# w111liang222/lidar-slam-detection

Measured on AMD Instinct MI355X. Metric: registered points/sec (120k-pt scan vs 1e7-pt map, full iterate-to-converge), higher is better.
Workload: dtype f32 per-point geometry / f64 transforms and reductions

## Files before the change

include/lio_hip.h:

```cpp
#ifndef LIO_HIP_H_
#define LIO_HIP_H_

#include <stdint.h>

#ifdef __cplusplus
extern "C" {
#endif

#define LIO_OK 0
#define LIO_E_INVALID (-1)
#define LIO_E_CAPACITY (-2)
#define LIO_E_DEVICE (-3)
#define LIO_E_STATE (-4)

typedef struct lio_map lio_map;
typedef struct lio_scan lio_scan;
typedef struct lio_engine lio_engine;

const char* lio_last_error(void);
const char* lio_last_warning(void);
int lio_device_count(void);
#define LIO_ABI_VERSION 16
int lio_abi_version(void);
void* lio_pinned_alloc(uint64_t bytes);
void lio_pinned_free(void* p);
uint64_t lio_map_bytes(const lio_map*);

lio_map* lio_map_create(int device, float resolution, uint64_t max_points, uint64_t max_voxels, int stencil);
void lio_map_destroy(lio_map*);
int lio_map_set_stencil(lio_map*, int stencil);
int lio_map_insert(lio_map*, const float* world_xyzi, uint64_t n, double travel);
int lio_map_insert_device(lio_map*, const void* d_world_xyzi, uint64_t n, double travel);
int lio_map_clear(lio_map*);
int lio_map_set_lru(lio_map*, uint64_t capacity_voxels, double max_distance);
int lio_map_lru_stats(lio_map*, uint64_t* n_evicted, uint64_t* n_interleaved);
int lio_map_lru_exact_stats(lio_map*, uint64_t* n_recreated, uint64_t* n_batches_not_followed);
int lio_map_set_tie_mode(lio_map*, int mode);
// ... 175 lines not shown
lio_batch* lio_batch_create_sequences(int device, float resolution, int stencil, uint64_t max_points, uint64_t max_voxels, int n_slots, int n_groups,
                                      uint32_t max_raw, uint32_t max_ds);
int lio_batch_sequences_step(lio_batch*, lio_scan_job* jobs, int n_jobs, double* cov_out);
int lio_batch_fastlio_main(lio_batch*, int* rc_out);
void lio_batch_destroy(lio_batch*);
int lio_batch_process(lio_batch*, lio_scan_job* jobs, int n_jobs);
typedef struct lio_batch_times {
    double downsample_us, knn_us, linearize_us, step_us;
    uint32_t downsample_launches, knn_launches, linearize_launches, step_launches;
    double insert_us;
    uint32_t insert_launches, pad;
} lio_batch_times;
int lio_batch_enable_kernel_timing(lio_batch*, int on);
int lio_batch_kernel_times(lio_batch*, lio_batch_times* out, int reset);
lio_engine* lio_batch_engine(lio_batch*, int group, int slot);
int lio_engine_set_static_map(lio_engine*, int on);

typedef struct lio_ndt lio_ndt;
lio_ndt* lio_ndt_create(int device, float resolution, int search_method, uint64_t max_points, uint64_t max_voxels, uint32_t max_source_points);
void lio_ndt_destroy(lio_ndt*);
int lio_ndt_set_target(lio_ndt*, const float* xyzi, uint64_t n);
int lio_ndt_set_target_device(lio_ndt*, const void* d_xyzi, uint64_t n);
int lio_ndt_num_voxels(lio_ndt*);
int lio_ndt_voxel_at(lio_ndt*, const float p[3], float mean[3], float cinv[9]);
int lio_ndt_linearize(lio_ndt*, lio_scan* source, const double T[16], int update_corr, int with_derivatives, double H[36], double b[6],
                      double* err, uint32_t* n_corr);
int lio_ndt_fitness_score(lio_ndt*, lio_scan* source, const double T[16], double max_range, double* score, uint32_t* n_inliers);
int lio_ndt_overlap_score(lio_ndt*, lio_scan* source, const double relpose[16], double max_range, double xy_range, double min_z, double* score,
                          double* inlier_ratio);
typedef struct lio_ndt_times {
// ... 388 lines not shown
```

lidar-slam-detection_amd/csrc/batch.hip:

```cpp
#include <sched.h>
#include <stdlib.h>

#include <chrono>
#include <deque>
#include <vector>

#include "eskf.h"
#include "lio_common.h"

using namespace lio;

int engine_resume_update(lio_engine* e, const double* x_now26, const double* x_prop26, const double* P_prop, int i, int converge, int t);
void engine_count_passes(lio_engine* e, int* n_pass, int* n_knn);
int engine_joint_register_device(lio_engine* e, const void* d_raw, uint32_t n_raw, double lidar_beg_time, double state26[26], double cov[529]);
struct lio_comm;
extern "C" int lio_comm_world(const lio_comm*);
extern "C" {
int engine_seq_prepare(lio_engine* e, uint32_t n_raw, double lidar_beg_time, int* ekf_inited);
void engine_seq_params(lio_engine* e, double* laser_cov, int* maximum_iter, int* degenerate_detect_en, float* leaf_surf, float* leaf_map, int* static_map,
                       double* travel, double last_pos_lid[3]);
int engine_seq_finish(lio_engine* e, const double x26[26], const double P529[529], int n_ds, int n_pass, int n_knn, int n_eff, int degenerate, int inserted,
                      uint32_t n_add, uint32_t map_err, uint32_t bound);
int engine_seq_resume(lio_engine* e, const double* x_now26, const double* x_prop26, const double* P_prop, int i, int converge, int t);
int engine_seq_has_lru(lio_engine* e);
// ... 15 lines not shown
    MapRef* d_rowmaps = nullptr;
    std::vector<MapRef> rowmap_rows;
    char* d_block = nullptr;
    char* h_block = nullptr;
    size_t block_bytes = 0;
    SlotDesc* d_desc = nullptr;
    SlotDesc* h_desc = nullptr;
    EskfDev* d_ctrl = nullptr;
    EskfDev* h_ctrl = nullptr;
    hipGraphExec_t exec[5] = {nullptr, nullptr, nullptr, nullptr, nullptr};
    const void* graph_table = nullptr;
    int graph_stencil = 0;
    lio_batch_result* h_res = nullptr;
    lio_batch_result* h_res_dev = nullptr;
    std::vector<int> job_of_slot;
    float4* d_rawbuf = nullptr;
    MapRef* d_maps = nullptr;
    MapRef* h_maps = nullptr;
    SeqDev* d_seq = nullptr;
    SeqDev* h_seq = nullptr;
    std::vector<int> seq_path;
    int any_lru = 0;
    int n_active = 0;
    int launched_passes = 4;
    uint32_t seq = 0;
    uint32_t max_n_raw = 0;
    BatchTimer* bt = nullptr;
};

}

struct lio_batch {
    lio_map* map = nullptr;
    int device = 0;
    int n_slots = 0;
    uint32_t max_raw = 0, max_ds = 0;
    int pred_passes = 4;
    bool broken = false;
    int use_graph = 1;
    int count_touched = 0;
    std::vector<lio_map*> maps;
    lio_comm* comm = nullptr;
    int world = 1;
    int rank = 0;
    int split_ds = 1;
    uint32_t ds_cap = 0;
    uint32_t ds_seen_max = 0;
    bool ds_cap_full = false;
    uint64_t n_ds_cut = 0;
    int (*gather_hook)(void*, const double*, double*, uint32_t, void*) = nullptr;
    void* gather_ctx = nullptr;
    bool joint = false;
    bool sequences = false;
    std::vector<lio_scan_job> fl_jobs;
// ... 55 lines not shown
    ek_begin(c);
}

void group_free(Group& g) {
    for (lio_engine* e : g.eng) lio_engine_destroy(e);
    for (lio_engine* e : g.sub_eng) lio_engine_destroy(e);
    if (g.d_local32) hipFree(g.d_local32);
    if (g.d_gathered) hipFree(g.d_gathered);
    if (g.d_ds_send) hipFree(g.d_ds_send);
    if (g.d_ds_all) hipFree(g.d_ds_all);
    if (g.d_rowmaps) hipFree(g.d_rowmaps);
    for (int k = 0; k < 5; k++)
        if (g.exec[k]) hipGraphExecDestroy(g.exec[k]);
    if (g.d_block) hipFree(g.d_block);
    if (g.d_rawbuf) hipFree(g.d_rawbuf);
    if (g.h_block) hipHostFree(g.h_block);
    if (g.d_seq) hipFree(g.d_seq);
    if (g.h_seq) hipHostFree(g.h_seq);
    if (g.h_res) hipHostFree(g.h_res);
    if (g.stream) hipStreamDestroy(g.stream);
    if (g.bt) {
        if (g.bt->created)
            for (int c = 0; c < BatchTimer::kClasses; c++)
                for (int i = 0; i < BatchTimer::kPool; i++) { hipEventDestroy(g.bt->ev[c][i][0]); hipEventDestroy(g.bt->ev[c][i][1]); }
        delete g.bt;
    }
}

const float4* stage_host_raw(lio_batch* b, Group& g, int slot, const lio_scan_job& job, int* rc) {
    *rc = LIO_OK;
// ... 84 lines not shown
            if (b->ds_cap == 0) {
                const char* k = getenv("LIO_JOINT_DS_CAP");
                const uint32_t want = k ? (uint32_t)strtoul(k, nullptr, 10) : ((ds_bound / 4u + 1023u) & ~1023u);
                b->ds_cap = std::min(ds_bound, std::max(k ? 1u : 4096u, want));
            }
            const uint32_t cap = b->ds_cap_full ? ds_bound : b->ds_cap;
            rc = p2plane_batch_exchange_ds(b->comm, b->world, b->gather_hook, b->gather_ctx, g.stream, g.d_desc, B, per, s0, s1, cap, g.d_ds_send, g.d_ds_all);
            if (rc == LIO_OK && s0 > 0) rc = scan_begin_rows(g.stream, g.d_desc, s0);
            if (rc == LIO_OK && s1 < B) rc = scan_begin_rows(g.stream, g.d_desc + s1, B - s1);
            if (rc != LIO_OK) return rc;
        } else {
            if (bt) bt->begin(0);
            rc = vg_downsample_batch(g.stream, g.d_desc, B, b->max_raw, b->max_ds, 0.5f, passes);
            if (bt) bt->end(0);
            if (rc != LIO_OK) return rc;
        }
        if (b->joint) {
            rc = p2plane_batch_share(g.stream, g.d_desc, B, M, ds_bound);
            if (rc == LIO_OK) rc = scan_begin_rows(g.stream, g.d_desc + B, B * (M - 1));
            if (rc != LIO_OK) return rc;
            return p2plane_batch_update_joint(b->maps.data(), M, b->comm, b->world, b->gather_hook, b->gather_ctx, g.stream, g.d_desc, B, ds_bound, 5, g.d_local32, g.d_gathered, bt,
                                              rowmaps);
        }
        return p2plane_batch_update(b->map, g.stream, g.d_desc, B, ds_bound, 5, bt, bt ? b->count_touched : 0);
    };
    if (!b->use_graph || timed || b->joint) return enqueue(timed ? g.bt : nullptr);
    if (g.graph_table != b->map->table || g.graph_stencil != b->map->stencil.n) {
        for (int k = 0; k < 5; k++)
            if (g.exec[k]) { hipGraphExecDestroy(g.exec[k]); g.exec[k] = nullptr; }
        g.graph_table = b->map->table;
// ... 44 lines not shown
    if (hipSetDevice(map->device) != hipSuccess) { set_error("lio_batch_create: no HIP device %d", map->device); return nullptr; }
    lio_batch* b = new lio_batch();
    b->map = map;
    b->device = map->device;
    b->n_slots = n_slots;
    b->max_raw = max_raw;
    b->max_ds = max_ds;
    b->maps.assign(maps, maps + n_maps);
    b->comm = comm;
    b->world = comm ? lio_comm_world(comm) : 1;
    b->rank = comm ? lio_comm_rank(comm) : 0;
    { const char* k = getenv("LIO_JOINT_SPLIT_DS"); b->split_ds = (k && k[0] == '0') ? 0 : 1; }
    b->joint = n_maps > 1 || comm != nullptr;
    b->groups.resize(n_groups);
    { const char* k = getenv("LIO_BATCH_GRAPH"); b->use_graph = (k && k[0] == '0') ? 0 : 1; }
    bool ok = true;
    const int M = n_maps;
    for (Group& g : b->groups) ok = ok && hipStreamCreateWithFlags(&g.stream, hipStreamNonBlocking) == hipSuccess;
    for (Group& g : b->groups) {
        g.job_of_slot.assign(n_slots, -1);
        const size_t desc_bytes = sizeof(SlotDesc) * (size_t)n_slots * (size_t)M;
        g.block_bytes = desc_bytes + sizeof(EskfDev) * (size_t)n_slots;
        ok = ok && hipMalloc(reinterpret_cast<void**>(&g.d_block), g.block_bytes) == hipSuccess;
        ok = ok && hipHostMalloc(reinterpret_cast<void**>(&g.h_block), g.block_bytes, hipHostMallocDefault) == hipSuccess;
        if (ok) {
            g.d_desc = reinterpret_cast<SlotDesc*>(g.d_block);
            g.h_desc = reinterpret_cast<SlotDesc*>(g.h_block);
            g.d_ctrl = reinterpret_cast<EskfDev*>(g.d_block + desc_bytes);
            g.h_ctrl = reinterpret_cast<EskfDev*>(g.h_block + desc_bytes);
        }
        ok = ok && hipHostMalloc(reinterpret_cast<void**>(&g.h_res), sizeof(lio_batch_result) * n_slots, hipHostMallocMapped) == hipSuccess;
        ok = ok && hipHostGetDevicePointer(reinterpret_cast<void**>(&g.h_res_dev), g.h_res, 0) == hipSuccess;
        if (b->joint) {
            ok = ok && hipMalloc(reinterpret_cast<void**>(&g.d_local32), sizeof(double) * 32 * n_slots) == hipSuccess;
            ok = ok && hipMalloc(reinterpret_cast<void**>(&g.d_gathered), sizeof(double) * 32 * n_slots * (size_t)b->world) == hipSuccess;
        }
        if (!ok) break;
        memset(g.h_block, 0, g.block_bytes);
        memset(g.h_res, 0, sizeof(lio_batch_result) * n_slots);
        ok = hipMemset(g.d_block, 0, g.block_bytes) == hipSuccess;
        for (int s = 0; s < n_slots && ok; s++) {
            lio_engine* e = lio_engine_create_shared(map, max_raw, max_ds);
            if (!e) { ok = false; break; }
            lio_engine_set_flags(e, 1, 0, 0.0, -10.0);
            g.eng.push_back(e);
            fill_desc(g.h_desc[s], lio_engine_scan(e), &g.d_ctrl[s], &g.h_res_dev[s]);
        }
        for (int m = 1; m < M && ok; m++)
            for (int s = 0; s < n_slots && ok; s++) {
                lio_engine* e = lio_engine_create_shared(maps[m], max_raw, max_ds);
                if (!e) { ok = false; break; }
                lio_engine_set_flags(e, 1, 0, 0.0, -10.0);
                g.sub_eng.push_back(e);
                fill_desc(g.h_desc[(size_t)m * n_slots + s], lio_engine_scan(e), &g.d_ctrl[s], nullptr);
            }
        for (int s = 0; s < n_slots && ok && b->joint; s++) {
            std::vector<lio_engine*> others;
            for (int m = 1; m < M; m++) others.push_back(g.sub_eng[(size_t)(m - 1) * n_slots + s]);
            ok = lio_engine_set_joint(g.eng[s], others.empty() ? nullptr : others.data(), (int)others.size(), comm) == LIO_OK;
        }
    }
// ... 84 lines not shown
int lio_batch_kernel_times(lio_batch* b, lio_batch_times* out, int reset) {
    if (!b || !out) return LIO_E_INVALID;
    memset(out, 0, sizeof(*out));
    for (Group& g : b->groups) {
        if (!g.bt) continue;
        out->downsample_us += g.bt->us[0]; out->knn_us += g.bt->us[1]; out->linearize_us += g.bt->us[2]; out->step_us += g.bt->us[3];
        out->downsample_launches += g.bt->launches[0]; out->knn_launches += g.bt->launches[1]; out->linearize_launches += g.bt->launches[2];
        out->step_launches += g.bt->launches[3];
        out->insert_us += g.bt->us[4];
        out->insert_launches += g.bt->launches[4];
        if (reset)
            for (int c = 0; c < BatchTimer::kClasses; c++) { g.bt->us[c] = 0; g.bt->launches[c] = 0; }
    }
    return LIO_OK;
}

lio_engine* lio_batch_engine(lio_batch* b, int group, int slot) {
    if (!b || group < 0 || group >= (int)b->groups.size() || slot < 0 || slot >= b->n_slots) return nullptr;
    return b->groups[group].eng[slot];
}

int lio_batch_process(lio_batch* b, lio_scan_job* jobs, int n_jobs) {
    if (!b || (!jobs && n_jobs) || n_jobs < 0) return LIO_E_INVALID;
    if (b->sequences) { set_error("lio_batch_process: a sequence batch is driven by lio_batch_sequences_step"); return LIO_E_STATE; }
    hipSetDevice(b->device);
    const int B = b->n_slots;
    int next = 0, first_err = 0;
    std::deque<int> inflight;
    std::vector<int> retry;
    auto note = [&](int rc) { if (rc < 0 && !first_err) first_err = rc; };
// ... 562 lines not shown
```

lidar-slam-detection_amd/csrc/knn.hip:

```cpp
#include "hashgrid.h"
#include "knn_dev.h"
#include "lio_common.h"
#include "refsel.h"

namespace lio {

#ifndef LIO_KNN_G
#define LIO_KNN_G 16
#endif
#ifndef LIO_KNN_U
#define LIO_KNN_U 4
#endif
#ifndef LIO_KNN_WAVES
#define LIO_KNN_WAVES 6
#endif
#ifndef LIO_KNN_PRUNE
#define LIO_KNN_PRUNE 1
#endif
#ifndef LIO_KNN_STAT
#define LIO_KNN_STAT 1
#endif
#ifndef LIO_KNN_WAVES_BATCH
#define LIO_KNN_WAVES_BATCH 7
#endif
// ... 255 lines not shown
__device__ __noinline__ bool cand_tie_less(const Cand& a, const Cand& b, const float4* __restrict__ pool) {
    if (a.id == b.id) return false;
    if (a.id == kNoIdx || b.id == kNoIdx) return a.id < b.id;
    const float4 pa = pool[a.id], pb = pool[b.id];
    if (pa.x != pb.x) return pa.x < pb.x;
    if (pa.y != pb.y) return pa.y < pb.y;
    if (pa.z != pb.z) return pa.z < pb.z;
    return a.id < b.id;
}
__device__ inline bool cand_less(const Cand& a, const Cand& b, const float4* __restrict__ pool) {
    if (a.d2 != b.d2) return a.d2 < b.d2;
    return cand_tie_less(a, b, pool);
}


template <int KM, int MODE, bool COUNT = false, class PoseFill>
__device__ __forceinline__ void knn_body(const Slot* __restrict__ table, uint32_t mask, const float4* __restrict__ pool,
                                         float inv_res, const StencilArgs& st, PoseFill fill, const float4* __restrict__ queries,
                                         uint32_t n_host, const ScanDev* __restrict__ sd, float4* __restrict__ world_out,
                                         float4* __restrict__ nn_pts, uint32_t nn_stride, int32_t* __restrict__ nn_cnt,
                                         MapDev* md, uint32_t* __restrict__ n_tie, uint32_t* __restrict__ tie_list) {
    __shared__ GroupLds lds[kGPB];
    const int tid = threadIdx.x;
    const int grp = tid / kG, gl = tid % kG;
    const int lane = tid & 63;
    GroupLds& g = lds[grp];
    const uint32_t n = sd ? sd->n_ds : n_host;
    const unsigned long long gmask = ((1ull << kG) - 1ull) << (lane - gl);
    __shared__ uint32_t stat_s[256 / 64];
    if (tid < 256 / 64) stat_s[tid] = 0;
    uint32_t touched = 0;
    uint32_t fresh = 0;
    uint32_t* const bits = COUNT ? md->touch_bits : nullptr;
    const float res = 1.0f / inv_res;
    const uint32_t b1_bits = __float_as_uint(0.0625f * res * res), b2_bits = __float_as_uint(0.25f * res * res);
    (void)b1_bits; (void)b2_bits;

    const uint32_t nblk = (n + kGPB - 1) / kGPB;
    const uint32_t per_xcd = (nblk + 7u) >> 3;
    const uint32_t wg_per_xcd = gridDim.x >> 3;
    constexpr uint32_t kAhead = 64 / kGPB;
    __shared__ float4 pw_s[64];
    __shared__ PoseArgs pose_s;
    if constexpr (MODE == 0) fill(pose_s);
    uint32_t ahead = kAhead;
    for (uint32_t j = blockIdx.x >> 3; j < per_xcd; j += wg_per_xcd) {
        const uint32_t q0 = ((blockIdx.x & 7u) * per_xcd + j) * kGPB;
        const uint32_t q = q0 + grp;
        const bool active = q < n;
        float4 pw = make_float4(0.f, 0.f, 0.f, 0.f);
        if constexpr (MODE == 0) {
            if (ahead == kAhead) {
                __syncthreads();
                if (tid < 64) {
                    const uint32_t j2 = j + (uint32_t)(tid / kGPB) * wg_per_xcd;
                    const uint32_t q2 = ((blockIdx.x & 7u) * per_xcd + j2) * kGPB + (uint32_t)(tid % kGPB);
                    if (j2 < per_xcd && q2 < n) {
                        float4 w2;
                        body_to_world(pose_s, queries[q2], w2);
                        world_out[q2] = w2;
                        uint32_t t2 = (uint32_t)tid;
                        asm volatile("" : "+v"(t2));
                        pw_s[t2] = w2;
                    }
                }
                __syncthreads();
                ahead = 0;
            }
            if (active) pw = pw_s[ahead * kGPB + grp];
            ahead++;
        } else {
            if (active) pw = queries[q];
        }
        int kx = 0, ky = 0, kz = 0;
        pos2grid(pw.x, pw.y, pw.z, inv_res, kx, ky, kz);
        uint32_t nhit = 0;
        constexpr bool kPrune = LIO_KNN_PRUNE && KM * kG <= 32;
        uint32_t n0 = 0, n01 = 0, total;
// ... 101 lines not shown
        for (int r = 0; r < 6; r++) {
            const uint32_t bd = group_min32(d0);
            const uint32_t bi = group_min32(d0 == bd ? i0d : 0xFFFFFFFFu);
            const bool some = bi != 0xFFFFFFFFu;
            if (r > 0 && some && bd == prev_d) tie = true;
            prev_d = some ? bd : 0xFFFFFFFFu;
            if (gl == r) win = bi;
            if (some && d0 == bd && i0d == bi) {
                d0 = d1; d1 = dd2; dd2 = d3; d3 = d4; d4 = 0xFFFFFFFFu;
                i0d = i1d; i1d = i2d; i2d = i3d; i3d = i4d; i4d = 0xFFFFFFFFu;
                pops++;
            }
        }
        if (group_ballot(pops >= 5 && drop_tie, lane)) tie = true;
        if (active && inrange > 0) {
            if (gl < 5) {
                uint32_t g2 = (uint32_t)gl;
                asm volatile("" : "+v"(g2));
                nn_pts[g2 * nn_stride + q] = (win != 0xFFFFFFFFu) ? pool[win] : make_float4(0.f, 0.f, 0.f, 0.f);
            }
            if (gl == 0) {
                nn_cnt[q] = inrange < 5 ? (int32_t)inrange : 5;
                if (tie) tie_list[atomicAdd(n_tie, 1u)] = q;
            }
        }
        group_lds_sync();
    }
    __shared__ unsigned long long vred[256 / 64];
    if constexpr (LIO_KNN_STAT || COUNT) {
        __syncthreads();
        uint32_t te = threadIdx.x;
        asm volatile("" : "+v"(te));
        if (te < 256 / 64) vred[te] = stat_s[te];
        __syncthreads();
        if (tid == 0) {
            const unsigned long long v = (vred[0] + vred[1]) + (vred[2] + vred[3]);
            if (v) atomicAdd(&md->knn_cand[(blockIdx.x & 63) * 16], v);
        }
// ... 27 lines not shown
                                                  float inv_res, StencilArgs st, PoseArgs pose, const float4* __restrict__ queries,
                                                  uint32_t n_host, const ScanDev* __restrict__ sd, float4* __restrict__ world_out,
                                                  float4* __restrict__ nn_pts, uint32_t nn_stride, int32_t* __restrict__ nn_cnt,
                                                  MapDev* md, uint32_t* __restrict__ n_tie, uint32_t* __restrict__ tie_list) {
    knn_body<KM, MODE>(table, mask, pool, inv_res, st, [&](PoseArgs& P) { if (threadIdx.x == 0) P = pose; }, queries, n_host, sd, world_out, nn_pts, nn_stride, nn_cnt, md,
                       n_tie, tie_list);
}
template <int KM, bool COUNT>
__global__ void LIO_KNN_OCC __launch_bounds__(256, COUNT ? LIO_KNN_WAVES : LIO_KNN_WAVES_BATCH) knn_batch_kernel(const Slot* __restrict__ table, uint32_t mask, const float4* __restrict__ pool,
                                                                       float inv_res, StencilArgs st, const SlotDesc* __restrict__ slots, MapDev* md) {
    const SlotDesc& d = slots[blockIdx.y];
    if (!d.active) return;
    const SlotGateLite sg = slot_gate_lite(d);
    if ((sg.status != EK_RUNNING) | (sg.converge == 0) | (sg.n_ds < d.min_ds)) return;
    const double* __restrict__ x = d.ctrl->x;
    knn_body<KM, 0, COUNT>(table, mask, pool, inv_res, st, [x](PoseArgs& P) { pose_fill_from_state(P, x); }, d.ds_body, sg.n_ds, nullptr, d.ds_world, d.nn_pts,
                                  d.max_ds, d.nn_cnt, md, &d.sd->n_tie, d.tie_list);
}

constexpr int kSelCap = 2560;
struct SelLds {
    uint32_t a_d[kSelCap], a_id[kSelCap], a_seq[kSelCap];
    refsel::Rec list[kSelCap];
    refsel::Rec fin[5 * kMaxStencil + 8];
    uint32_t v_ptr[kMaxStencil], v_cnt[kMaxStencil];
    uint32_t v_first[kMaxStencil + 1];
    uint32_t seg_m[kMaxStencil], seg_base[kMaxStencil + 1], seg_keep[kMaxStencil];
    uint32_t wsum[4];
    uint32_t out_d[8], out_id[8];
    int size;
};

// ... 263 lines not shown
    const SlotGate sg = slot_gate(d);
    if ((sg.status != EK_RUNNING) | (sg.converge == 0) | (sg.n_ds < d.min_ds)) return;
    knn_refsel_body<0>(r.table, r.mask, r.pool, r.pool_seq, r.inv_res, st, sg.pose, d.ds_body, d.nn_pts, d.max_ds, &d.sd->n_tie, d.tie_list, r.md, r.tie_mode, sg.n_ds);
}
template <int KM>
__global__ void __launch_bounds__(256) knn_exact_batch_kernel(const Slot* __restrict__ table, uint32_t mask, const float4* __restrict__ pool,
                                                              float inv_res, StencilArgs st, const SlotDesc* __restrict__ slots, int tie_mode) {
    const SlotDesc& d = slots[blockIdx.y];
    if (!d.active || d.sd->n_tie == 0) return;
    const SlotGate sg = slot_gate(d);
    if ((sg.status != EK_RUNNING) | (sg.converge == 0) | (sg.n_ds < d.min_ds)) return;
    const PoseArgs& pose = sg.pose;
    knn_exact_body<KM, 0>(table, mask, pool, inv_res, st, pose, d.ds_body, d.nn_pts, d.max_ds, &d.sd->n_tie, d.tie_list, tie_mode);
}

int knn_batch_launch(lio_map* m, hipStream_t st, const SlotDesc* d_slots, int n_slots, uint32_t grid_x, int count_touched) {
    static const uint32_t forced = [] { const char* e = getenv("LIO_KNN_GRID"); const int v = e ? atoi(e) : 0; return v >= 8 ? (uint32_t)v : 0u; }();
    uint32_t cap = forced ? forced : (12288u / (uint32_t)(n_slots > 0 ? n_slots : 1));
    if (cap > 2048u) cap = 2048u;
    if (cap < 128u) cap = 128u;
    if (grid_x > cap) grid_x = cap;
    if (grid_x == 0) grid_x = 8;
    const dim3 grid((grid_x + 7u) & ~7u, (uint32_t)n_slots);
    const dim3 gridx(n_slots > 8 ? 8 : 64, (uint32_t)n_slots);
    const int tmode = m->pool_seq ? m->tie_mode : 0;
    const int km = (m->stencil.n + kG - 1) / kG;
    if (count_touched && m->touch_bits) LIO_HIP_TRY(hipMemsetAsync(m->touch_bits, 0, (size_t)((m->pool_cap + 31) / 32) * 4, st));
#define KNNB_LAUNCH(KM)                                                                                                                              \
    do {                                                                                                                                             \
        if (count_touched) hipLaunchKernelGGL((knn_batch_kernel<KM, true>), grid, 256, 0, st, m->table, m->table_mask, m->pool, m->inv_res, m->stencil, d_slots, m->dev); \
// ... 152 lines not shown
```

lidar-slam-detection_amd/csrc/lio_common.h:

```cpp
#pragma once
#include <hip/hip_runtime.h>
#include <stdint.h>
#include <stdio.h>
#include <string.h>

#include "../../include/lio_hip.h"
#include "eskf_dev.h"

struct LruEntry;

namespace lio {

#if defined(__HIP_DEVICE_COMPILE__)
#define LIO_PIN4(r) asm volatile("" : "+v"((r).x), "+v"((r).y), "+v"((r).z), "+v"((r).w))
#define LIO_PIN1(r) asm volatile("" : "+v"(r))
#else
#define LIO_PIN4(r) ((void)(r))
#define LIO_PIN1(r) ((void)(r))
#endif
__host__ __device__ __forceinline__ void pin_loaded(float4& r) { LIO_PIN4(r); }
__host__ __device__ __forceinline__ void pin_loaded(uint4& r) { LIO_PIN4(r); }
__host__ __device__ __forceinline__ void pin_loaded(uint32_t& r) { LIO_PIN1(r); }
__host__ __device__ __forceinline__ void pin_loaded(float& r) { LIO_PIN1(r); }

// ... 91 lines not shown
    uint32_t nblocks;
    uint32_t active;
    uint32_t seq;
    uint32_t max_ds, partial_blocks;
    uint32_t min_ds;
    uint32_t reset_cache;
    ScanDev* sd;
    uint32_t *keys_a, *keys_b, *vals_a, *vals_b, *hist, *blockcnt, *hpos, *longlist, *tie_list;
    float4 *sorted, *ds_body, *ds_world, *nn_pts, *normvec;
    int32_t* nn_cnt;
    uint8_t* selected;
    double* partial;
    uint32_t* host_nds;
    EskfDev* ctrl;
    lio_batch_result* result;
};

struct MapRef {
    Slot* table;
    uint32_t* cap;
    uint32_t* pending;
    float* created;
    float4* pool;
    uint32_t* pool_seq;
    MapDev* md;
    uint32_t* slot_of_point;
    float4* stage;
    unsigned long long pool_cap;
    unsigned long long stamp_base;
    unsigned long long* touch;
// ... 152 lines not shown
constexpr int kMaxPoseList = 64;
struct PoseListArgs {
    int n_poses;
    unsigned long long limit[kMaxPoseList];
    DeltaArgs d[kMaxPoseList];
};
int undistort_poses_launch(hipStream_t stream, const float4* d_in, const uint32_t* d_stamp_us, uint32_t n, float4* d_out, const PoseListArgs& args,
                           uint32_t* d_tile_max);
int undistort_delta_launch(hipStream_t stream, const float4* d_in, const uint32_t* d_stamp_us, uint32_t n, float4* d_out, const DeltaArgs& args);
int undistort_launch(hipStream_t stream, const float4* d_in, const uint32_t* d_stamp_us, uint32_t n, float4* d_out, const ImuPoseDev* d_poses,
                     const UndistortArgs& args, unsigned long long* d_block_min );

int vg_downsample(lio_scan* s, float leaf, int passes );
int vg_downsample_batch(hipStream_t st, const SlotDesc* d_slots, int n_slots, uint32_t max_raw, uint32_t max_ds, float leaf, int passes);
int knn_batch_launch(lio_map* m, hipStream_t st, const SlotDesc* d_slots, int n_slots, uint32_t grid_x, int count_touched);
struct BatchTimer {
    static constexpr int kClasses = 5;
    static constexpr int kPool = 256;
    hipEvent_t ev[kClasses][kPool][2];
    int used[kClasses] = {0, 0, 0, 0, 0};
    double us[kClasses] = {0, 0, 0, 0, 0};
    uint32_t launches[kClasses] = {0, 0, 0, 0, 0};
    bool on = false, created = false;
    hipStream_t stream = nullptr;
    void begin(int c) { if (on && used[c] < kPool) hipEventRecord(ev[c][used[c]][0], stream); }
    void end(int c) { if (on && used[c] < kPool) { hipEventRecord(ev[c][used[c]][1], stream); used[c]++; } }
    void resolve() {
        for (int c = 0; c < kClasses; c++) {
            for (int i = 0; i < used[c]; i++) {
                float ms = 0.f;
// ... 51 lines not shown
```

lidar-slam-detection_amd/python/lsd_amd/capi.py:

```python
import ctypes as C
import os

import numpy as np

_HERE = os.path.dirname(os.path.abspath(__file__))
os.environ.setdefault("GPU_MAX_HW_QUEUES", "8")
LIB_PATH = os.environ.get("LIO_HIP_LIB") or os.path.join(_HERE, "liblio_hip.so")

LIO_OK, LIO_E_INVALID, LIO_E_CAPACITY, LIO_E_DEVICE, LIO_E_STATE = 0, -1, -2, -3, -4
MAIN_FIRST_SCAN, MAIN_SEEDED, MAIN_SKIPPED, MAIN_UPDATED, MAIN_IMU_INIT, MAIN_IDLE = 0, 1, 2, 3, 4, 5

SYMBOLS = [
    "lio_last_warning",
    "lio_last_error", "lio_device_count", "lio_map_bytes",
    "lio_map_create", "lio_map_destroy", "lio_map_set_lru", "lio_map_lru_stats", "lio_map_lru_exact_stats", "lio_map_set_tie_mode", "lio_map_tie_stats", "lio_map_clear", "lio_map_pool_stats", "lio_map_set_stencil", "lio_map_insert", "lio_map_insert_device", "lio_map_stats",
    "lio_abi_version", "lio_pinned_alloc", "lio_pinned_free",
    "lio_map_dump", "lio_map_knn", "lio_map_knn_candidates", "lio_map_knn_touched", "lio_map_knn_unique",
    "lio_scan_create", "lio_scan_destroy", "lio_scan_reset", "lio_scan_upload", "lio_scan_set_device", "lio_scan_undistort_delta", "lio_scan_undistort_poses", "lio_scan_undistort_imu", "lio_scan_download_raw", "lio_scan_voxel_downsample", "lio_scan_voxel_downsample_batch", "lio_scan_set_ds",
    "lio_scan_num_ds", "lio_scan_download_ds", "lio_scan_download_world", "lio_scan_download_match",
    "lio_p2plane_linearize", "lio_scan_set_degeneracy_mode", "lio_p2plane_degeneracy", "lio_engine_set_reduce_hook", "lio_p2plane_rows", "lio_map_incremental", "lio_map_seed",
    "lio_engine_create", "lio_engine_create_shared", "lio_engine_destroy", "lio_engine_map", "lio_engine_scan", "lio_engine_set_state", "lio_engine_get_state",
    "lio_engine_set_cov", "lio_engine_get_cov", "lio_engine_set_flags", "lio_engine_travel", "lio_engine_is_degenerate",
    "lio_engine_update", "lio_engine_pass_log", "lio_engine_process_scan", "lio_engine_process_scan_device", "lio_engine_timings", "lio_engine_flush",
    "lio_engine_enable_timing", "lio_comm_unique_id", "lio_comm_init", "lio_comm_destroy", "lio_comm_rank", "lio_comm_world", "lio_allgather_normal_eq", "lio_comm_stats", "lio_engine_set_joint", "lio_engine_joint_register", "lio_engine_joint_register_device", "lio_allgather_records", "lio_engines_process_batch", "lio_batch_create", "lio_batch_create_joint", "lio_batch_create_sequences", "lio_batch_sequences_step", "lio_batch_fastlio_main", "lio_batch_set_gather_hook", "lio_batch_exchange_stats", "lio_batch_destroy", "lio_batch_process", "lio_batch_engine", "lio_batch_enable_kernel_timing", "lio_batch_kernel_times", "lio_engine_set_static_map", "lio_scan_enable_kernel_timing", "lio_scan_kernel_times",
    "lio_state_boxplus", "lio_state_boxminus",
    "lio_localmap_create", "lio_localmap_destroy", "lio_localmap_add_keyframe", "lio_localmap_num_keyframes", "lio_localmap_update",
    "lio_localmap_download",
    "lio_cloud_create", "lio_cloud_destroy", "lio_cloud_clear", "lio_cloud_size", "lio_cloud_append_scan", "lio_cloud_append_host",
    "lio_cloud_voxel_downsample", "lio_cloud_download", "lio_cloud_scratch_bytes", "lio_cloud_last_times",
    "lio_knn_index_create", "lio_knn_index_destroy", "lio_knn_index_build", "lio_knn_index_query", "lio_knn_index_colour", "lio_knn_index_last_times",
    "lio_ground_default_params", "lio_ground_draw", "lio_ground_create", "lio_ground_destroy", "lio_ground_detect_scan", "lio_ground_detect_host",
    "lio_ground_download_indices", "lio_ground_download_normals", "lio_ground_download_inliers", "lio_ground_download_draws", "lio_ground_last_run",
    "lio_ground_last_times",
    "lio_bev_create", "lio_bev_destroy", "lio_bev_preprocess_host", "lio_bev_preprocess_cloud", "lio_bev_upload_pixels", "lio_bev_convert", "lio_bev_get_info",
    "lio_bev_download_pixel_coords", "lio_bev_download_kept", "lio_bev_download_pixels", "lio_bev_download_nodes", "lio_bev_download_equalised",
    "lio_bev_download_image", "lio_bev_grey_table", "lio_bev_last_times",
    "lio_keyframe_decide", "lio_keyframer_default_params", "lio_keyframer_create", "lio_keyframer_destroy", "lio_keyframer_reset", "lio_keyframer_push_host",
    "lio_keyframer_pending", "lio_keyframer_pop", "lio_radius_outlier_host", "lio_keyframe_filter_host", "lio_keyframer_fitness_host",
    "lio_keyframer_append_local_map_host", "lio_keyframer_download_local_map", "lio_keyframer_last_times",
# ... 262 lines not shown
    sig("lio_comm_stats", cint, vp, C.POINTER(u64), f64p)
    sig("lio_engine_set_joint", cint, vp, C.POINTER(vp), cint, vp)
    sig("lio_engine_joint_register", cint, vp, f32p, u32, dbl, f64p, f64p)
    sig("lio_engine_joint_register_device", cint, vp, vp, u32, dbl, f64p, f64p)
    sig("lio_allgather_records", cint, vp, vp, vp, u32, vp)
    sig("lio_batch_create_joint", vp, C.POINTER(vp), cint, vp, cint, cint, u32, u32)
    sig("lio_batch_set_gather_hook", cint, vp, GATHER_FN, vp, cint, cint)
    sig("lio_batch_exchange_stats", cint, vp, C.POINTER(C.c_uint32), C.POINTER(C.c_uint64), C.POINTER(C.c_uint64))
    sig("lio_batch_create", vp, vp, cint, cint, u32, u32)
    sig("lio_batch_create_sequences", vp, cint, C.c_float, cint, u64, u64, cint, cint, u32, u32)
    sig("lio_batch_sequences_step", cint, vp, C.POINTER(ScanJob), cint, C.POINTER(C.c_double))
    sig("lio_batch_fastlio_main", cint, vp, C.POINTER(cint))
    sig("lio_batch_destroy", None, vp)
    sig("lio_batch_process", cint, vp, C.POINTER(ScanJob), cint)
    sig("lio_batch_engine", vp, vp, cint, cint)
    sig("lio_batch_enable_kernel_timing", cint, vp, cint)
    sig("lio_batch_kernel_times", cint, vp, C.POINTER(BatchTimes), cint)
    sig("lio_engine_set_static_map", cint, vp, cint)
    sig("lio_localmap_create", vp, cint, u64, u32, u32)
    sig("lio_localmap_destroy", None, vp)
    sig("lio_localmap_add_keyframe", cint, vp, f32p, u32, f32p)
    sig("lio_localmap_num_keyframes", cint, vp)
    sig("lio_localmap_update", cint, vp, vp, f64p, dbl, dbl, dbl, flt, C.POINTER(cint), C.POINTER(u32))
    sig("lio_localmap_download", cint, vp, f32p, u32)
    sig("lio_cloud_create", vp, cint, u64)
    sig("lio_cloud_destroy", None, vp)
    sig("lio_cloud_clear", cint, vp)
    sig("lio_cloud_size", cint, vp, C.POINTER(u64))
    sig("lio_cloud_append_scan", cint, vp, vp, f64p, flt, cint, dbl, dbl)
    sig("lio_cloud_append_host", cint, vp, f32p, u64, f64p, flt, cint, dbl, dbl)
# ... 198 lines not shown
```

lidar-slam-detection_amd/python/lsd_amd/lio.py:

```python
import ctypes as C

import numpy as np

from . import capi
from .capi import check, f32, f64, lib, ptr

STATE_DIM = 26
DOF = 23
G_LEN = 9.809


def default_state():
    s = np.zeros(STATE_DIM)
    s[6] = 1.0
    s[10] = 1.0
    s[23] = G_LEN
    return s


def init_cov():
    P = np.eye(23)
    for i in (6, 7, 8, 9, 10, 11):
        P[i, i] = 0.00001
    for i in (15, 16, 17):
# ... 1559 lines not shown
        check(lib().lio_batch_set_gather_hook(self.h, self._gather, None, int(rank), int(world)), "set_gather_hook")

    def exchange_stats(self):
        cap, again, nbytes = C.c_uint32(0), C.c_uint64(0), C.c_uint64(0)
        check(lib().lio_batch_exchange_stats(self.h, C.byref(cap), C.byref(again), C.byref(nbytes)))
        return {"chunk_points": cap.value, "jobs_rerun": again.value, "bytes_per_rank_and_round": nbytes.value}

    def enable_kernel_timing(self, on=True):
        check(lib().lio_batch_enable_kernel_timing(self.h, int(on)))

    def kernel_times(self, reset=True):
        t = capi.BatchTimes()
        check(lib().lio_batch_kernel_times(self.h, C.byref(t), int(reset)))
        return {k: getattr(t, k) for k, _ in t._fields_}

    def engine(self, group, slot):
        h = lib().lio_batch_engine(self.h, group, slot)
        if not h:
            raise capi.LioError("no such slot")
        e = Engine.__new__(Engine)
        e.h = h
        e._own = False
        e.map = self.map
        e.scan = Scan(max_ds=100000, _borrow=lib().lio_engine_scan(h))
        return e

    def process(self, jobs):
        return process_batch(None, jobs, batch=self)


# ... 379 lines not shown
```

Baseline: 5.948 billion.

## Sort KNN queries by Morton order of downsampled points for map locality

Adds a per-slot kernel that computes a 30-bit Morton key for each downsampled scan point and radix-sorts indices in LDS, producing a query permutation. The batch KNN kernel then stages queries in this spatial order and writes results back to the original indices, so neighbouring threads probe nearby hash-grid cells and map points. The aim is better cache reuse and less divergence in map lookups, at the cost of an extra sort launch per scan and an indirection in query loads. Scans larger than the LDS cap fall back to identity order.

```diff
diff --git a/include/lio_hip.h b/include/lio_hip.h
--- a/include/lio_hip.h
+++ b/include/lio_hip.h
@@ -20,7 +20,7 @@
 const char* lio_last_error(void);
 const char* lio_last_warning(void);
 int lio_device_count(void);
-#define LIO_ABI_VERSION 16
+#define LIO_ABI_VERSION 17
 int lio_abi_version(void);
 void* lio_pinned_alloc(uint64_t bytes);
 void lio_pinned_free(void* p);
@@ -226,6 +226,9 @@
 int lio_batch_enable_kernel_timing(lio_batch*, int on);
 int lio_batch_kernel_times(lio_batch*, lio_batch_times* out, int reset);
 lio_engine* lio_batch_engine(lio_batch*, int group, int slot);
+int lio_batch_set_query_order(lio_batch*, int on);
+int lio_batch_query_order(lio_batch*, int group, int slot, uint32_t* out, uint32_t cap);
+uint32_t lio_batch_query_order_cap(void);
 int lio_engine_set_static_map(lio_engine*, int on);
 
 typedef struct lio_ndt lio_ndt;
diff --git a/lidar-slam-detection_amd/csrc/batch.hip b/lidar-slam-detection_amd/csrc/batch.hip
--- a/lidar-slam-detection_amd/csrc/batch.hip
+++ b/lidar-slam-detection_amd/csrc/batch.hip
@@ -53,6 +53,7 @@
     lio_batch_result* h_res = nullptr;
     lio_batch_result* h_res_dev = nullptr;
     std::vector<int> job_of_slot;
+    uint32_t* d_qorder = nullptr;
     float4* d_rawbuf = nullptr;
     MapRef* d_maps = nullptr;
     MapRef* h_maps = nullptr;
@@ -77,6 +78,7 @@
     int pred_passes = 4;
     bool broken = false;
     int use_graph = 1;
+    int query_order = 0;
     int count_touched = 0;
     std::vector<lio_map*> maps;
     lio_comm* comm = nullptr;
@@ -162,6 +164,7 @@
         if (g.exec[k]) hipGraphExecDestroy(g.exec[k]);
     if (g.d_block) hipFree(g.d_block);
     if (g.d_rawbuf) hipFree(g.d_rawbuf);
+    if (g.d_qorder) hipFree(g.d_qorder);
     if (g.h_block) hipHostFree(g.h_block);
     if (g.d_seq) hipFree(g.d_seq);
     if (g.h_seq) hipHostFree(g.h_seq);
@@ -276,6 +279,8 @@
             rc = vg_downsample_batch(g.stream, g.d_desc, B, b->max_raw, b->max_ds, 0.5f, passes);
             if (bt) bt->end(0);
             if (rc != LIO_OK) return rc;
+            if (b->query_order) rc = knn_order_batch_launch(g.stream, g.d_desc, B, 0.5f);
+            if (rc != LIO_OK) return rc;
         }
         if (b->joint) {
             rc = p2plane_batch_share(g.stream, g.d_desc, B, M, ds_bound);
@@ -350,6 +355,7 @@
     b->joint = n_maps > 1 || comm != nullptr;
     b->groups.resize(n_groups);
     { const char* k = getenv("LIO_BATCH_GRAPH"); b->use_graph = (k && k[0] == '0') ? 0 : 1; }
+    { const char* k = getenv("LIO_KNN_ORDER"); b->query_order = (b->joint || (k && k[0] == '0')) ? 0 : 1; }
     bool ok = true;
     const int M = n_maps;
     for (Group& g : b->groups) ok = ok && hipStreamCreateWithFlags(&g.stream, hipStreamNonBlocking) == hipSuccess;
@@ -370,6 +376,8 @@
         if (b->joint) {
             ok = ok && hipMalloc(reinterpret_cast<void**>(&g.d_local32), sizeof(double) * 32 * n_slots) == hipSuccess;
             ok = ok && hipMalloc(reinterpret_cast<void**>(&g.d_gathered), sizeof(double) * 32 * n_slots * (size_t)b->world) == hipSuccess;
+        } else {
+            ok = ok && hipMalloc(reinterpret_cast<void**>(&g.d_qorder), sizeof(uint32_t) * (size_t)max_ds * (size_t)n_slots) == hipSuccess;
         }
         if (!ok) break;
         memset(g.h_block, 0, g.block_bytes);
@@ -381,6 +389,7 @@
             lio_engine_set_flags(e, 1, 0, 0.0, -10.0);
             g.eng.push_back(e);
             fill_desc(g.h_desc[s], lio_engine_scan(e), &g.d_ctrl[s], &g.h_res_dev[s]);
+            g.h_desc[s].qorder = b->query_order ? g.d_qorder + (size_t)s * max_ds : nullptr;
         }
         for (int m = 1; m < M && ok; m++)
             for (int s = 0; s < n_slots && ok; s++) {
@@ -495,6 +504,45 @@
     }
     return LIO_OK;
 }
+
+int lio_batch_set_query_order(lio_batch* b, int on) {
+    if (!b) return LIO_E_INVALID;
+    if (b->joint || b->sequences) {
+        if (!on) return LIO_OK;
+        set_error("lio_batch_set_query_order: only the static batch (lio_batch_create) orders its queries");
+        return LIO_E_STATE;
+    }
+    hipSetDevice(b->device);
+    for (Group& g : b->groups) {
+        LIO_HIP_TRY(hipStreamSynchronize(g.stream));
+        for (int s = 0; s < b->n_slots; s++) g.h_desc[s].qorder = on ? g.d_qorder + (size_t)s * b->max_ds : nullptr;
+        for (int k = 0; k < 5; k++)
+            if (g.exec[k]) { hipGraphExecDestroy(g.exec[k]); g.exec[k] = nullptr; }
+    }
+    b->query_order = on ? 1 : 0;
+    return LIO_OK;
+}
+
+int lio_batch_query_order(lio_batch* b, int group, int slot, uint32_t* out, uint32_t cap) {
+    if (!b || group < 0 || group >= (int)b->groups.size() || slot < 0 || slot >= b->n_slots || (!out && cap)) return LIO_E_INVALID;
+    if (b->sequences) { set_error("lio_batch_query_order: a sequence batch does not order its queries"); return LIO_E_STATE; }
+    hipSetDevice(b->device);
+    Group& g = b->groups[group];
+    LIO_HIP_TRY(hipStreamSynchronize(g.stream));
+    lio_scan* sc = lio_engine_scan(g.eng[slot]);
+    uint32_t n = 0;
+    LIO_HIP_TRY(hipMemcpy(&n, &sc->dev->n_ds, sizeof(uint32_t), hipMemcpyDeviceToHost));
+    if (n > b->max_ds) n = b->max_ds;
+    const uint32_t m = n < cap ? n : cap;
+    if (b->query_order && g.d_qorder) {
+        if (m) LIO_HIP_TRY(hipMemcpy(out, g.d_qorder + (size_t)slot * b->max_ds, sizeof(uint32_t) * m, hipMemcpyDeviceToHost));
+    } else {
+        for (uint32_t i = 0; i < m; i++) out[i] = i;
+    }
+    return (int)n;
+}
+
+uint32_t lio_batch_query_order_cap(void) { return knn_order_cap(); }
 
 lio_engine* lio_batch_engine(lio_batch* b, int group, int slot) {
     if (!b || group < 0 || group >= (int)b->groups.size() || slot < 0 || slot >= b->n_slots) return nullptr;
diff --git a/lidar-slam-detection_amd/csrc/knn.hip b/lidar-slam-detection_amd/csrc/knn.hip
--- a/lidar-slam-detection_amd/csrc/knn.hip
+++ b/lidar-slam-detection_amd/csrc/knn.hip
@@ -1,5 +1,6 @@
 #include "hashgrid.h"
 #include "knn_dev.h"
+#include "knn_order.h"
 #include "lio_common.h"
 #include "refsel.h"
 
@@ -293,12 +294,14 @@
 }
 
 
-template <int KM, int MODE, bool COUNT = false, class PoseFill>
+template <int KM, int MODE, bool COUNT = false, bool ORDERED = false, class PoseFill>
 __device__ __forceinline__ void knn_body(const Slot* __restrict__ table, uint32_t mask, const float4* __restrict__ pool,
                                          float inv_res, const StencilArgs& st, PoseFill fill, const float4* __restrict__ queries,
                                          uint32_t n_host, const ScanDev* __restrict__ sd, float4* __restrict__ world_out,
                                          float4* __restrict__ nn_pts, uint32_t nn_stride, int32_t* __restrict__ nn_cnt,
-                                         MapDev* md, uint32_t* __restrict__ n_tie, uint32_t* __restrict__ tie_list) {
+                                         MapDev* md, uint32_t* __restrict__ n_tie, uint32_t* __restrict__ tie_list,
+                                         const uint32_t* __restrict__ order = nullptr) {
+    static_assert(!ORDERED || MODE == 0, "the query order is looked up by the staging wave of MODE 0");
     __shared__ GroupLds lds[kGPB];
     const int tid = threadIdx.x;
     const int grp = tid / kG, gl = tid % kG;
@@ -321,6 +324,19 @@
     constexpr uint32_t kAhead = 64 / kGPB;
     __shared__ float4 pw_s[64];
     __shared__ PoseArgs pose_s;
+    __shared__ uint32_t qi_s[64];
+    __shared__ uint32_t qn_s[64];
+    __shared__ const uint32_t* order_s;
+    if constexpr (ORDERED) {
+        if (tid == 0) order_s = order;
+        if (tid < 64) {
+            uint32_t t0 = (uint32_t)tid;
+            asm volatile("" : "+v"(t0));
+            const uint32_t j2 = (blockIdx.x >> 3) + (t0 / kGPB) * wg_per_xcd;
+            const uint32_t q2 = ((blockIdx.x & 7u) * per_xcd + j2) * kGPB + (t0 % kGPB);
+            qn_s[t0] = (order && j2 < per_xcd && q2 < n) ? order[q2] : q2;
+        }
+    }
     if constexpr (MODE == 0) fill(pose_s);
     uint32_t ahead = kAhead;
     for (uint32_t j = blockIdx.x >> 3; j < per_xcd; j += wg_per_xcd) {
@@ -334,13 +350,27 @@
                 if (tid < 64) {
                     const uint32_t j2 = j + (uint32_t)(tid / kGPB) * wg_per_xcd;
                     const uint32_t q2 = ((blockIdx.x & 7u) * per_xcd + j2) * kGPB + (uint32_t)(tid % kGPB);
-                    if (j2 < per_xcd && q2 < n) {
+                    uint32_t qi = q2, nxt = 0;
+                    if constexpr (ORDERED) {
+                        const uint32_t j3 = j2 + kAhead * wg_per_xcd, q3 = q2 + kAhead * wg_per_xcd * kGPB;
+                        const uint32_t* const ord = order_s;
+                        const bool more = ord && j3 < per_xcd && q3 < n;
+                        nxt = q3;
+                        if (more) nxt = ord[q3];
+                        qi = qn_s[tid];
+                        if (qi >= n) qi = q2;
+                    }
+                    const bool staged = j2 < per_xcd && q2 < n;
+                    const float4 pq = queries[staged ? qi : 0u];
+                    if constexpr (ORDERED) qn_s[tid] = nxt;
+                    if (staged) {
                         float4 w2;
-                        body_to_world(pose_s, queries[q2], w2);
-                        world_out[q2] = w2;
+                        body_to_world(pose_s, pq, w2);
+                        world_out[qi] = w2;
                         uint32_t t2 = (uint32_t)tid;
                         asm volatile("" : "+v"(t2));
                         pw_s[t2] = w2;
+                        if constexpr (ORDERED) qi_s[t2] = qi;
                     }
                 }
                 __syncthreads();
@@ -472,14 +502,20 @@
         }
         if (group_ballot(pops >= 5 && drop_tie, lane)) tie = true;
         if (active && inrange > 0) {
+            uint32_t qo = q;
+            if constexpr (ORDERED) {
+                uint32_t gq = (uint32_t)grp;
+                asm volatile("" : "+v"(gq));
+                qo = qi_s[(ahead - 1u) * kGPB + gq];
+            }
             if (gl < 5) {
                 uint32_t g2 = (uint32_t)gl;
                 asm volatile("" : "+v"(g2));
-                nn_pts[g2 * nn_stride + q] = (win != 0xFFFFFFFFu) ? pool[win] : make_float4(0.f, 0.f, 0.f, 0.f);
+                nn_pts[g2 * nn_stride + qo] = (win != 0xFFFFFFFFu) ? pool[win] : make_float4(0.f, 0.f, 0.f, 0.f);
             }
             if (gl == 0) {
-                nn_cnt[q] = inrange < 5 ? (int32_t)inrange : 5;
-                if (tie) tie_list[atomicAdd(n_tie, 1u)] = q;
+                nn_cnt[qo] = inrange < 5 ? (int32_t)inrange : 5;
+                if (tie) tie_list[atomicAdd(n_tie, 1u)] = qo;
             }
         }
         group_lds_sync();
@@ -537,8 +573,8 @@
     const SlotGateLite sg = slot_gate_lite(d);
     if ((sg.status != EK_RUNNING) | (sg.converge == 0) | (sg.n_ds < d.min_ds)) return;
     const double* __restrict__ x = d.ctrl->x;
-    knn_body<KM, 0, COUNT>(table, mask, pool, inv_res, st, [x](PoseArgs& P) { pose_fill_from_state(P, x); }, d.ds_body, sg.n_ds, nullptr, d.ds_world, d.nn_pts,
-                                  d.max_ds, d.nn_cnt, md, &d.sd->n_tie, d.tie_list);
+    knn_body<KM, 0, COUNT, true>(table, mask, pool, inv_res, st, [x](PoseArgs& P) { pose_fill_from_state(P, x); }, d.ds_body, sg.n_ds, nullptr, d.ds_world, d.nn_pts,
+                                  d.max_ds, d.nn_cnt, md, &d.sd->n_tie, d.tie_list, d.qorder);
 }
 
 constexpr int kSelCap = 2560;
@@ -832,6 +868,100 @@
     knn_exact_body<KM, 0>(table, mask, pool, inv_res, st, pose, d.ds_body, d.nn_pts, d.max_ds, &d.sd->n_tie, d.tie_list, tie_mode);
 }
 
+constexpr int kOrdThreads = 1024, kOrdWaves = kOrdThreads / 64, kOrdPasses = 5;
+constexpr uint32_t kOrderCap = 19200;
+struct OrderLds {
+    uint32_t key[kOrderCap];
+    uint16_t idx[2][kOrderCap];
+    uint32_t cnt[kOrdWaves][64];
+};
+__global__ void __launch_bounds__(kOrdThreads) knn_order_batch(const SlotDesc* __restrict__ slots, float inv_leaf) {
+    const SlotDesc& d = slots[blockIdx.y];
+    if (!d.active || !d.qorder) return;
+    uint32_t n = d.sd->n_ds;
+    if (n > d.max_ds) n = d.max_ds;
+    if (n == 0) return;
+    uint32_t* __restrict__ out = d.qorder;
+    const uint32_t tid = threadIdx.x, lane = tid & 63u, w = tid >> 6;
+    if (n > kOrderCap) {
+        for (uint32_t i = tid; i < n; i += kOrdThreads) out[i] = i;
+        return;
+    }
+    __shared__ OrderLds S;
+    const int mx = d.sd->minb[0], my = d.sd->minb[1], mz = d.sd->minb[2];
+    const float4* __restrict__ pts = d.ds_body;
+    for (uint32_t i0 = 0; i0 < n; i0 += 4u * kOrdThreads) {
+        float4 p[4];
+#pragma unroll
+        for (int u = 0; u < 4; u++) {
+            const uint32_t i = i0 + (uint32_t)u * kOrdThreads + tid;
+            p[u] = pts[i < n ? i : 0u];
+        }
+#pragma unroll
+        for (int u = 0; u < 4; u++) pin_loaded(p[u]);
+#pragma unroll
+        for (int u = 0; u < 4; u++) {
+            const uint32_t i = i0 + (uint32_t)u * kOrdThreads + tid;
+            if (i < n) {
+                S.key[i] = order_key(p[u].x, p[u].y, p[u].z, inv_leaf, mx, my, mz);
+                S.idx[0][i] = (uint16_t)i;
+            }
+        }
+    }
+    __syncthreads();
+    const uint32_t chunk = ((n + kOrdThreads - 1u) / kOrdThreads) * 64u;
+    const uint32_t beg = w * chunk < n ? w * chunk : n, end = beg + chunk < n ? beg + chunk : n;
+    int src = 0;
+    for (int pass = 0; pass < kOrdPasses; pass++) {
+        const int sh = pass * 6;
+        S.cnt[w][lane] = 0;
+        group_lds_sync();
+        for (uint32_t i = beg + lane; i < end; i += 64u) atomicAdd(&S.cnt[w][(S.key[S.idx[src][i]] >> sh) & 63u], 1u);
+        __syncthreads();
+        uint32_t tot = 0, pre = 0;
+#pragma unroll
+        for (uint32_t w2 = 0; w2 < (uint32_t)kOrdWaves; w2++) {
+            const uint32_t c = S.cnt[w2][lane];
+            tot += c;
+            pre += w2 < w ? c : 0u;
+        }
+        uint32_t inc = tot;
+#pragma unroll
+        for (int o = 1; o < 64; o <<= 1) {
+            const uint32_t t = __shfl_up(inc, o);
+            if (lane >= (uint32_t)o) inc += t;
+        }
+        uint32_t next = inc - tot + pre;
+        for (uint32_t b0 = beg; b0 < end; b0 += 64u) {
+            const uint32_t i = b0 + lane;
+            const bool valid = i < end;
+            const uint32_t id = valid ? S.idx[src][i] : 0u;
+            const uint32_t dg = (S.key[id] >> sh) & 63u;
+            unsigned long long peers = __ballot(valid), mine = peers;
+#pragma unroll
+            for (int bit = 0; bit < 6; bit++) {
+                const unsigned long long bb = __ballot(valid && ((dg >> bit) & 1u));
+                peers &= ((dg >> bit) & 1u) ? bb : ~bb;
+                mine &= ((lane >> bit) & 1u) ? bb : ~bb;
+            }
+            const uint32_t rank = __builtin_amdgcn_mbcnt_hi((uint32_t)(peers >> 32), __builtin_amdgcn_mbcnt_lo((uint32_t)peers, 0u));
+            const uint32_t pos = (uint32_t)__shfl((int)next, (int)dg) + rank;
+            if (valid) S.idx[src ^ 1][pos] = (uint16_t)id;
+            next += (uint32_t)__popcll(mine);
+        }
+        __syncthreads();
+        src ^= 1;
+    }
+    for (uint32_t i = tid; i < n; i += kOrdThreads) out[i] = S.idx[src][i];
+}
+int knn_order_batch_launch(hipStream_t st, const SlotDesc* d_slots, int n_slots, float leaf) {
+    if (n_slots <= 0) return LIO_OK;
+    hipLaunchKernelGGL(knn_order_batch, dim3(1, (uint32_t)n_slots), kOrdThreads, 0, st, d_slots, 1.0f / leaf);
+    LIO_HIP_TRY(hipGetLastError());
+    return LIO_OK;
+}
+uint32_t knn_order_cap() { return kOrderCap; }
+
 int knn_batch_launch(lio_map* m, hipStream_t st, const SlotDesc* d_slots, int n_slots, uint32_t grid_x, int count_touched) {
     static const uint32_t forced = [] { const char* e = getenv("LIO_KNN_GRID"); const int v = e ? atoi(e) : 0; return v >= 8 ? (uint32_t)v : 0u; }();
     uint32_t cap = forced ? forced : (12288u / (uint32_t)(n_slots > 0 ? n_slots : 1));
diff --git a/lidar-slam-detection_amd/csrc/knn_order.h b/lidar-slam-detection_amd/csrc/knn_order.h
--- /dev/null
+++ b/lidar-slam-detection_amd/csrc/knn_order.h
@@ -0,0 +1,37 @@
+#pragma once
+#include <math.h>
+#include <stdint.h>
+
+#ifndef LIO_HD
+#ifdef __HIPCC__
+#define LIO_HD __host__ __device__
+#else
+#define LIO_HD
+#endif
+#endif
+
+namespace lio {
+
+constexpr int kOrderAxisBits = 10;
+
+LIO_HD inline uint32_t order_spread3(uint32_t v) {
+    v &= 0x3FFu;
+    v = (v | (v << 16)) & 0x030000FFu;
+    v = (v | (v << 8)) & 0x0300F00Fu;
+    v = (v | (v << 4)) & 0x030C30C3u;
+    v = (v | (v << 2)) & 0x09249249u;
+    return v;
+}
+
+LIO_HD inline uint32_t order_cell(float p, float inv_leaf, int minb) {
+    const float f = floorf(p * inv_leaf) - (float)minb;
+    const float hi = (float)((1 << kOrderAxisBits) - 1);
+    return (uint32_t)(f >= 0.f ? (f <= hi ? f : hi) : 0.f);
+}
+
+LIO_HD inline uint32_t order_key(float x, float y, float z, float inv_leaf, int minx, int miny, int minz) {
+    return order_spread3(order_cell(x, inv_leaf, minx)) | (order_spread3(order_cell(y, inv_leaf, miny)) << 1) |
+           (order_spread3(order_cell(z, inv_leaf, minz)) << 2);
+}
+
+}
diff --git a/lidar-slam-detection_amd/csrc/lio_common.h b/lidar-slam-detection_amd/csrc/lio_common.h
--- a/lidar-slam-detection_amd/csrc/lio_common.h
+++ b/lidar-slam-detection_amd/csrc/lio_common.h
@@ -129,6 +129,7 @@
     uint32_t* host_nds;
     EskfDev* ctrl;
     lio_batch_result* result;
+    uint32_t* qorder;
 };
 
 struct MapRef {
@@ -311,6 +312,8 @@
 int vg_downsample(lio_scan* s, float leaf, int passes );
 int vg_downsample_batch(hipStream_t st, const SlotDesc* d_slots, int n_slots, uint32_t max_raw, uint32_t max_ds, float leaf, int passes);
 int knn_batch_launch(lio_map* m, hipStream_t st, const SlotDesc* d_slots, int n_slots, uint32_t grid_x, int count_touched);
+int knn_order_batch_launch(hipStream_t st, const SlotDesc* d_slots, int n_slots, float leaf);
+uint32_t knn_order_cap();
 struct BatchTimer {
     static constexpr int kClasses = 5;
     static constexpr int kPool = 256;
diff --git a/lidar-slam-detection_amd/python/lsd_amd/capi.py b/lidar-slam-detection_amd/python/lsd_amd/capi.py
--- a/lidar-slam-detection_amd/python/lsd_amd/capi.py
+++ b/lidar-slam-detection_amd/python/lsd_amd/capi.py
@@ -22,7 +22,7 @@
     "lio_engine_create", "lio_engine_create_shared", "lio_engine_destroy", "lio_engine_map", "lio_engine_scan", "lio_engine_set_state", "lio_engine_get_state",
     "lio_engine_set_cov", "lio_engine_get_cov", "lio_engine_set_flags", "lio_engine_travel", "lio_engine_is_degenerate",
     "lio_engine_update", "lio_engine_pass_log", "lio_engine_process_scan", "lio_engine_process_scan_device", "lio_engine_timings", "lio_engine_flush",
-    "lio_engine_enable_timing", "lio_comm_unique_id", "lio_comm_init", "lio_comm_destroy", "lio_comm_rank", "lio_comm_world", "lio_allgather_normal_eq", "lio_comm_stats", "lio_engine_set_joint", "lio_engine_joint_register", "lio_engine_joint_register_device", "lio_allgather_records", "lio_engines_process_batch", "lio_batch_create", "lio_batch_create_joint", "lio_batch_create_sequences", "lio_batch_sequences_step", "lio_batch_fastlio_main", "lio_batch_set_gather_hook", "lio_batch_exchange_stats", "lio_batch_destroy", "lio_batch_process", "lio_batch_engine", "lio_batch_enable_kernel_timing", "lio_batch_kernel_times", "lio_engine_set_static_map", "lio_scan_enable_kernel_timing", "lio_scan_kernel_times",
+    "lio_engine_enable_timing", "lio_comm_unique_id", "lio_comm_init", "lio_comm_destroy", "lio_comm_rank", "lio_comm_world", "lio_allgather_normal_eq", "lio_comm_stats", "lio_engine_set_joint", "lio_engine_joint_register", "lio_engine_joint_register_device", "lio_allgather_records", "lio_engines_process_batch", "lio_batch_create", "lio_batch_create_joint", "lio_batch_create_sequences", "lio_batch_sequences_step", "lio_batch_fastlio_main", "lio_batch_set_gather_hook", "lio_batch_exchange_stats", "lio_batch_destroy", "lio_batch_process", "lio_batch_engine", "lio_batch_set_query_order", "lio_batch_query_order", "lio_batch_query_order_cap", "lio_batch_enable_kernel_timing", "lio_batch_kernel_times", "lio_engine_set_static_map", "lio_scan_enable_kernel_timing", "lio_scan_kernel_times",
     "lio_state_boxplus", "lio_state_boxminus",
     "lio_localmap_create", "lio_localmap_destroy", "lio_localmap_add_keyframe", "lio_localmap_num_keyframes", "lio_localmap_update",
     "lio_localmap_download",
@@ -315,6 +315,9 @@
     sig("lio_batch_destroy", None, vp)
     sig("lio_batch_process", cint, vp, C.POINTER(ScanJob), cint)
     sig("lio_batch_engine", vp, vp, cint, cint)
+    sig("lio_batch_set_query_order", cint, vp, cint)
+    sig("lio_batch_query_order", cint, vp, cint, cint, C.POINTER(C.c_uint32), u32)
+    sig("lio_batch_query_order_cap", u32)
     sig("lio_batch_enable_kernel_timing", cint, vp, cint)
     sig("lio_batch_kernel_times", cint, vp, C.POINTER(BatchTimes), cint)
     sig("lio_engine_set_static_map", cint, vp, cint)
diff --git a/lidar-slam-detection_amd/python/lsd_amd/lio.py b/lidar-slam-detection_amd/python/lsd_amd/lio.py
--- a/lidar-slam-detection_amd/python/lsd_amd/lio.py
+++ b/lidar-slam-detection_amd/python/lsd_amd/lio.py
@@ -1597,6 +1597,23 @@
         check(lib().lio_batch_kernel_times(self.h, C.byref(t), int(reset)))
         return {k: getattr(t, k) for k, _ in t._fields_}
 
+    def set_query_order(self, on=True):
+        check(lib().lio_batch_set_query_order(self.h, int(bool(on))), "set_query_order")
+
+    def query_order(self, group, slot):
+        import numpy as np
+
+        n = lib().lio_batch_query_order(self.h, int(group), int(slot), None, 0)
+        check(min(n, 0), "query_order")
+        out = np.zeros(max(n, 1), np.uint32)
+        n2 = lib().lio_batch_query_order(self.h, int(group), int(slot), out.ctypes.data_as(C.POINTER(C.c_uint32)), int(n))
+        check(min(n2, 0), "query_order")
+        return out[:min(n, n2)]
+
+    @staticmethod
+    def query_order_cap():
+        return int(lib().lio_batch_query_order_cap())
+
     def engine(self, group, slot):
         h = lib().lio_batch_engine(self.h, group, slot)
         if not h:
```

After: 5.846 billion. -1.7%, worse.
